# wenyuqing/panacea

Measured on NVIDIA H100. Metric: UNet denoise-steps/s (6-view x 8-frame latent, CFG-doubled eps-eval + guidance + Euler update), higher is better.
Workload: dtype bf16

## Files before the change

### panacea_b200/csrc/attn_fa.cu

```cuda
#include "common.cuh"
#include "ptx.cuh"
#include "operand.cuh"
#include "../../include/panacea_b200.h"

namespace pn {

constexpr int FA_THREADS = 288;
constexpr int FA_TILE_BYTES = 128 * 128;
constexpr int FA_XTILE_BYTES = 128 * 32;
constexpr int FA_MAX_KEYS = 128;
constexpr int FA_QBOX = 8;

template <int D>
struct FaL {
  static constexpr int STAGES = 3;
  static constexpr int XB = D == 64 ? 0 : FA_XTILE_BYTES;
  static constexpr int Q = 0;
  static constexpr int QX = FA_TILE_BYTES;
  static constexpr int KV = FA_TILE_BYTES + XB;
  static constexpr int STAGE_BYTES = 2 * FA_TILE_BYTES + 2 * XB;
  static constexpr int BAR = KV + STAGES * STAGE_BYTES;
  static constexpr int TOTAL = BAR + 128 + 1024;
};

struct FaParams {
  CUtensorMap mapQ;
  CUtensorMap mapK;
  CUtensorMap mapV;
  CUtensorMap mapQx, mapKx, mapVx;
  int heads;
  int F, H, V, W;
  int q_rowmajor;
  int qw, qh, tiles_x, tiles_y;
  int tiles_per_group;
  int kw, kh, kv_rows, kv_yblocks;
  int kv_views[8][2];
  int kv_view_count[8];
  int kv_frame_div;
  float scale_log2;
  __nv_bfloat16* out;
  long long out_ld;
};

template <int D, int N>
__global__ void __launch_bounds__(FA_THREADS, 1) attn_fa_kernel(const __grid_constant__ FaParams p) {
  static_assert(N % 16 == 0 && N >= 16 && N <= FA_MAX_KEYS, "a key block is a whole number of K = 16 steps of P V");
  using L = FaL<D>;
  constexpr int STAGES = L::STAGES;
  constexpr int GROUPS = N / 8;
  constexpr int KSTEPS = N / 16;
  extern __shared__ uint8_t smem_raw[];
  uint8_t* smem = smem_align1024(smem_raw);
  uint64_t* bars = reinterpret_cast<uint64_t*>(smem + L::BAR);
  uint64_t* q_full = bars;
  uint64_t* kv_full = bars + 1;
  uint64_t* kv_empty = bars + 1 + STAGES;

  const int warp = threadIdx.x >> 5;
  const int lane = threadIdx.x & 31;

  {
    uint4* z = reinterpret_cast<uint4*>(smem);
    for (int i = threadIdx.x; i < L::BAR / 16; i += FA_THREADS) z[i] = make_uint4(0, 0, 0, 0);
    fence_proxy_async_smem();
  }
  if (threadIdx.x == 0) {
    mbar_init(q_full, 1);
    for (int i = 0; i < STAGES; ++i) { mbar_init(&kv_full[i], 1); mbar_init(&kv_empty[i], 2); }
    fence_barrier_init();
  }
  __syncthreads();

  int item = blockIdx.x;
  const int ti = item % p.tiles_per_group; item /= p.tiles_per_group;
  const int head = item % p.heads; item /= p.heads;
  const int view = item % p.V;
  const int frame = item / p.V;
  const int nblk = p.kv_view_count[view] * p.kv_yblocks;

  if (warp == 8) {
    const uint32_t row_bytes = D == 80 ? 160u : 128u;
    const uint32_t kv_bytes = (uint32_t)p.kv_rows * row_bytes;
    if (elect_one()) {
      tma_prefetch_desc(&p.mapQ);
      tma_prefetch_desc(&p.mapK);
      tma_prefetch_desc(&p.mapV);
      if (p.q_rowmajor) {
        const int t0 = ti * 128;
        const int rows = min(128, p.H * p.W - t0);
        mbar_arrive_expect_tx(q_full, (uint32_t)rows * row_bytes);
        for (int r = 0; r < rows; r += FA_QBOX) {
          const int y = (t0 + r) / p.W, x = t0 + r - y * p.W;
          tma_load_5d(smem + L::Q + r * 128, &p.mapQ, q_full, head * D, x, view, y, frame);
          if (D == 80) tma_load_5d(smem + L::QX + r * 32, &p.mapQx, q_full, head * D + 64, x, view, y, frame);
        }
      } else {
        mbar_arrive_expect_tx(q_full, (uint32_t)(p.qw * p.qh) * row_bytes);
        const int x0 = (ti % p.tiles_x) * p.qw, y0 = (ti / p.tiles_x) * p.qh;
        tma_load_5d(smem + L::Q, &p.mapQ, q_full, head * D, x0, view, y0, frame);
        if (D == 80) tma_load_5d(smem + L::QX, &p.mapQx, q_full, head * D + 64, x0, view, y0, frame);
      }
    }
    const int kv_frame = frame / p.kv_frame_div;
    int vi = 0, yb = 0;
    for (int j = 0; j < nblk; ++j) {
      const int st = j % STAGES;
      const int kvv = p.kv_views[view][vi];
      mbar_wait(&kv_empty[st], (uint32_t)(((j / STAGES) & 1) ^ 1));
      if (elect_one()) {
        uint8_t* sK = smem + L::KV + st * L::STAGE_BYTES;
        mbar_arrive_expect_tx(&kv_full[st], 2 * kv_bytes);
        tma_load_5d(sK, &p.mapK, &kv_full[st], head * D, 0, kvv, yb * p.kh, kv_frame);
        tma_load_5d(sK + FA_TILE_BYTES, &p.mapV, &kv_full[st], head * D, 0, kvv, yb * p.kh, kv_frame);
        if (D == 80) {
          tma_load_5d(sK + 2 * FA_TILE_BYTES, &p.mapKx, &kv_full[st], head * D + 64, 0, kvv, yb * p.kh, kv_frame);
          tma_load_5d(sK + 2 * FA_TILE_BYTES + L::XB, &p.mapVx, &kv_full[st], head * D + 64, 0, kvv, yb * p.kh, kv_frame);
        }
      }
      if (++yb == p.kv_yblocks) { yb = 0; ++vi; }
    }
    return;
  }

  const int wg = warp >> 2;
  const int quad = lane & 3;
  const uint32_t base = smem_u32(smem);
  const uint64_t dQ = wgmma_desc(base + L::Q + wg * 64 * 128, 16, 1024, kSw128);
  const uint64_t dQx = wgmma_desc(base + L::QX + wg * 64 * 32, 16, 256, kSw32);
  const uint64_t dK0 = wgmma_desc(base + L::KV, 16, 1024, kSw128);
  const uint64_t dV0 = wgmma_desc(base + L::KV + FA_TILE_BYTES, 1024, 1024, kSw128);
  const uint64_t dKx0 = wgmma_desc(base + L::KV + 2 * FA_TILE_BYTES, 16, 256, kSw32);
  const uint64_t dVx0 = wgmma_desc(base + L::KV + 2 * FA_TILE_BYTES + L::XB, 256, 256, kSw32);
  constexpr uint64_t STAGE_STEP = L::STAGE_BYTES >> 4;
  const float c = p.scale_log2;
  const bool mask = p.kv_rows < N;

  float o[32], ox[8];
#pragma unroll
  for (int i = 0; i < 32; ++i) o[i] = 0.f;
#pragma unroll
  for (int i = 0; i < 8; ++i) ox[i] = 0.f;
  float m_run[2] = {-INFINITY, -INFINITY}, l_run[2] = {0.f, 0.f};
  float s[N / 2];
  uint32_t pa[KSTEPS][4];
  float alpha[2];

  auto issue_s = [&](int st) {
#pragma unroll
    for (int k = 0; k < 4; ++k) wgmma_ss<N>(s, dQ + 2 * k, dK0 + STAGE_STEP * st + 2 * k, k > 0 ? 1u : 0u);
    if (D == 80) wgmma_ss<N>(s, dQx, dKx0 + STAGE_STEP * st, 1u);
    wgmma_commit();
  };
  auto issue_pv = [&](int st) {
#pragma unroll
    for (int kk = 0; kk < KSTEPS; ++kk) {
      wgmma_rs_tb<64>(o, pa[kk], dV0 + STAGE_STEP * st + kk * (2048 >> 4), 1u);
      if (D == 80) wgmma_rs_tb<16>(ox, pa[kk], dVx0 + STAGE_STEP * st + kk * (512 >> 4), 1u);
    }
    wgmma_commit();
  };
  auto softmax = [&]() {
    float mx[2] = {-INFINITY, -INFINITY};
#pragma unroll
    for (int jj = 0; jj < GROUPS; ++jj) {
#pragma unroll
      for (int e = 0; e < 4; ++e) {
        if (jj >= GROUPS - 2 && mask && 8 * jj + 2 * quad + (e & 1) >= p.kv_rows) s[4 * jj + e] = -INFINITY;
        mx[e >> 1] = fmaxf(mx[e >> 1], s[4 * jj + e]);
      }
    }
    float mc[2];
#pragma unroll
    for (int h = 0; h < 2; ++h) {
      mx[h] = fmaxf(mx[h], __shfl_xor_sync(0xffffffffu, mx[h], 1));
      mx[h] = fmaxf(mx[h], __shfl_xor_sync(0xffffffffu, mx[h], 2));
      const float m_new = fmaxf(m_run[h], mx[h]);
      alpha[h] = ex2_approx((m_run[h] - m_new) * c);
      m_run[h] = m_new;
      mc[h] = m_new * c;
    }
    float rs[2] = {0.f, 0.f};
#pragma unroll
    for (int jj = 0; jj < GROUPS; ++jj) {
#pragma unroll
      for (int e = 0; e < 4; ++e) {
        const float x = fmaf(s[4 * jj + e], c, -mc[e >> 1]);
        const float v = ex2_approx(x);
        s[4 * jj + e] = v;
        rs[e >> 1] += v;
      }
    }
#pragma unroll
    for (int h = 0; h < 2; ++h) l_run[h] = l_run[h] * alpha[h] + rs[h];
  };
  auto rescale_and_pack = [&]() {
#pragma unroll
    for (int i = 0; i < 32; ++i) o[i] *= alpha[(i >> 1) & 1];
    if (D == 80) {
#pragma unroll
      for (int i = 0; i < 8; ++i) ox[i] *= alpha[(i >> 1) & 1];
    }
#pragma unroll
    for (int jj = 0; jj < GROUPS; ++jj) {
#pragma unroll
      for (int h = 0; h < 2; ++h) pa[jj >> 1][(jj & 1) * 2 + h] = pack_bf16x2(s[4 * jj + 2 * h], s[4 * jj + 2 * h + 1]);
    }
  };
  auto pv_retired = [&](int st) {
    wgmma_fence_regs(o);
    if (D == 80) wgmma_fence_regs(ox);
#pragma unroll
    for (int kk = 0; kk < KSTEPS; ++kk) wgmma_fence_regs(pa[kk]);
    if ((threadIdx.x & 127) == 0) mbar_arrive(&kv_empty[st]);
  };

  mbar_wait(q_full, 0);
  mbar_wait(&kv_full[0], 0);
  wgmma_fence();
  issue_s(0);
  wgmma_wait<0>();
  wgmma_fence_regs(s);
  softmax();
  rescale_and_pack();
  for (int j = 1; j < nblk; ++j) {
    const int st = j % STAGES, prev = (j - 1) % STAGES;
    mbar_wait(&kv_full[st], (uint32_t)((j / STAGES) & 1));
    wgmma_fence();
    issue_s(st);
    issue_pv(prev);
    wgmma_wait<0>();
    wgmma_fence_regs(s);
    pv_retired(prev);
    softmax();
    rescale_and_pack();
  }
  wgmma_fence();
  issue_pv((nblk - 1) % STAGES);
  wgmma_wait<0>();
  pv_retired((nblk - 1) % STAGES);

#pragma unroll
  for (int h = 0; h < 2; ++h) {
    float l = l_run[h];
    l += __shfl_xor_sync(0xffffffffu, l, 1);
    l += __shfl_xor_sync(0xffffffffu, l, 2);
    const float inv = 1.f / l;
    const int row = wg * 64 + (warp & 3) * 16 + (lane >> 2) + 8 * h;
    int x, y;
    if (p.q_rowmajor) {
      const int t = ti * 128 + row;
      y = t / p.W;
      x = t - y * p.W;
    } else {
      if (row >= p.qw * p.qh) continue;
      const int yy = row / p.qw, xx = row - yy * p.qw;
      x = (ti % p.tiles_x) * p.qw + xx;
      y = (ti / p.tiles_x) * p.qh + yy;
    }
    if (x >= p.W || y >= p.H) continue;
    const long long token = (((long long)frame * p.H + y) * p.V + view) * p.W + x;
    __nv_bfloat16* dst = p.out + token * p.out_ld + head * D + 2 * quad;
#pragma unroll
    for (int jj = 0; jj < 8; ++jj)
      *reinterpret_cast<uint32_t*>(dst + 8 * jj) = pack_bf16x2(o[4 * jj + 2 * h] * inv, o[4 * jj + 2 * h + 1] * inv);
    if (D == 80) {
#pragma unroll
      for (int jj = 0; jj < 2; ++jj)
        *reinterpret_cast<uint32_t*>(dst + 64 + 8 * jj) = pack_bf16x2(ox[4 * jj + 2 * h] * inv, ox[4 * jj + 2 * h + 1] * inv);
    }
  }
}

template <int D>
void (*const fa_kernels[FA_MAX_KEYS / 16])(FaParams) = {attn_fa_kernel<D, 16>, attn_fa_kernel<D, 32>, attn_fa_kernel<D, 48>,
                                                        attn_fa_kernel<D, 64>, attn_fa_kernel<D, 80>, attn_fa_kernel<D, 96>,
                                                        attn_fa_kernel<D, 112>, attn_fa_kernel<D, 128>};

}

using namespace pn;

extern "C" int pn_attention(const pn_attn_args* a, int operand_mode, void* stream_v) {
  PN_OPERAND_MODES(Modes, operand_mode, "pn_attention", PN_OPERAND_BF16, PN_OPERAND_SPLIT3, PN_OPERAND_F32);
  if (operand_mode != PN_OPERAND_BF16) return attention_f32(a, operand_mode, stream_v);
  if (a == nullptr) return fail(PN_ERR_INVALID, "pn_attention: null args");
  PN_REQUIRE(a->q && a->k && a->v && a->out, "pn_attention: null tensor pointer");
  PN_REQUIRE(a->head_dim == 64 || a->head_dim == 80, "pn_attention: head_dim %d unsupported (64 or 80)", a->head_dim);
  const int FA_D = a->head_dim;
  PN_REQUIRE(a->heads > 0 && a->F > 0 && a->H > 0 && a->V > 0 && a->V <= 8 && a->W > 0, "pn_attention: bad query geometry");
  PN_REQUIRE(a->Hk > 0 && a->Vk > 0 && a->Vk <= 8 && a->Wk > 0 && a->kv_frame_div > 0, "pn_attention: bad key geometry");
  PN_REQUIRE(a->q_ld % 8 == 0 && a->kv_ld % 8 == 0 && a->out_ld % 8 == 0, "pn_attention: token strides must be multiples of 8");
  PN_REQUIRE(a->q_ld >= a->heads * FA_D && a->kv_ld >= a->heads * FA_D && a->out_ld >= a->heads * FA_D,
             "pn_attention: token stride smaller than heads*64");

  FaParams p;
  std::memset(&p, 0, sizeof(p));
  p.heads = a->heads;
  p.F = (int)a->F; p.H = (int)a->H; p.V = (int)a->V; p.W = (int)a->W;
  p.qw = (int)(a->W <= 128 ? a->W : 128);
  p.qh = 128 / p.qw;
  if (p.qh > a->H) p.qh = (int)a->H;
  if (p.qh < 1) p.qh = 1;
  p.tiles_x = (int)((a->W + p.qw - 1) / p.qw);
  p.tiles_y = (int)((a->H + p.qh - 1) / p.qh);
  p.q_rowmajor = a->W % FA_QBOX == 0 && a->W < 128 && p.qw * p.qh < 128 && a->H > p.qh;
  PN_REQUIRE(a->Wk <= FA_MAX_KEYS, "pn_attention: key view width %lld > %d unsupported", (long long)a->Wk, FA_MAX_KEYS);
  p.kw = (int)a->Wk;
  int kh = FA_MAX_KEYS / p.kw;
  if (kh > a->Hk) kh = (int)a->Hk;
  while (kh > 1 && (a->Hk % kh) != 0) --kh;
  p.kh = kh;
  p.kv_rows = p.kw * p.kh;
  p.kv_yblocks = (int)(a->Hk / p.kh);
  for (int v = 0; v < a->V; ++v) {
    const int cnt = a->kv_view_count[v];
    PN_REQUIRE(cnt >= 1 && cnt <= 2, "pn_attention: kv_view_count[%d]=%d must be 1 or 2", v, cnt);
    p.kv_view_count[v] = cnt;
    for (int i = 0; i < cnt; ++i) {
      PN_REQUIRE(a->kv_views[v][i] >= 0 && a->kv_views[v][i] < a->Vk, "pn_attention: kv view out of range");
      p.kv_views[v][i] = a->kv_views[v][i];
    }
  }
  p.kv_frame_div = a->kv_frame_div;
  p.scale_log2 = a->scale * 1.4426950408889634f;
  p.out = reinterpret_cast<__nv_bfloat16*>(a->out);
  p.out_ld = a->out_ld;

  const uint64_t chq = (uint64_t)a->heads * FA_D;
  {
    const uint64_t dims[5] = {chq, (uint64_t)a->W, (uint64_t)a->V, (uint64_t)a->H, (uint64_t)a->F};
    const uint64_t ld = (uint64_t)a->q_ld;
    const uint64_t str[4] = {ld, ld * a->W, ld * a->W * a->V, ld * a->W * a->V * a->H};
    const uint32_t bw = p.q_rowmajor ? FA_QBOX : p.qw, bh = p.q_rowmajor ? 1 : p.qh;
    const uint32_t box[5] = {64u, bw, 1u, bh, 1u};
    int rc = cached_tmap_bf16(&p.mapQ, a->q, 5, dims, str, box, 128);
    if (rc != PN_OK) return rc;
    if (FA_D == 80) {
      const uint32_t boxx[5] = {16u, bw, 1u, bh, 1u};
      rc = cached_tmap_bf16(&p.mapQx, a->q, 5, dims, str, boxx, 32);
      if (rc != PN_OK) return rc;
    }
  }
  {
    const uint64_t Fk = (uint64_t)((a->F + a->kv_frame_div - 1) / a->kv_frame_div);
    const uint64_t dims[5] = {chq, (uint64_t)a->Wk, (uint64_t)a->Vk, (uint64_t)a->Hk, Fk};
    const uint64_t ld = (uint64_t)a->kv_ld;
    const uint64_t str[4] = {ld, ld * a->Wk, ld * a->Wk * a->Vk, ld * a->Wk * a->Vk * a->Hk};
    const uint32_t box[5] = {64u, (uint32_t)p.kw, 1u, (uint32_t)p.kh, 1u};
    int rc = cached_tmap_bf16(&p.mapK, a->k, 5, dims, str, box, 128);
    if (rc != PN_OK) return rc;
    rc = cached_tmap_bf16(&p.mapV, a->v, 5, dims, str, box, 128);
    if (rc != PN_OK) return rc;
    if (FA_D == 80) {
      const uint32_t boxx[5] = {16u, (uint32_t)p.kw, 1u, (uint32_t)p.kh, 1u};
      rc = cached_tmap_bf16(&p.mapKx, a->k, 5, dims, str, boxx, 32);
      if (rc != PN_OK) return rc;
      rc = cached_tmap_bf16(&p.mapVx, a->v, 5, dims, str, boxx, 32);
      if (rc != PN_OK) return rc;
    }
  }
  p.tiles_per_group = p.q_rowmajor ? (int)((a->H * a->W + 127) / 128) : p.tiles_x * p.tiles_y;
  const long long items = (long long)p.tiles_per_group * a->heads * a->V * a->F;
  PN_REQUIRE(items > 0 && items < (1ll << 31), "pn_attention: too many query tiles");
  const int n_idx = (p.kv_rows + 15) / 16 - 1;
  void (*kern)(FaParams) = FA_D == 80 ? fa_kernels<80>[n_idx] : fa_kernels<64>[n_idx];
  const size_t smem_total = FA_D == 80 ? FaL<80>::TOTAL : FaL<64>::TOTAL;
  {
    const int rc = ensure_dyn_smem(reinterpret_cast<const void*>(kern), smem_total);
    if (rc != PN_OK) return rc;
  }
  kern<<<(unsigned)items, FA_THREADS, smem_total, reinterpret_cast<cudaStream_t>(stream_v)>>>(p);
  PN_CHECK_CUDA(cudaGetLastError());
  return PN_OK;
}
```

Measured before the change: 4.208.

## Make attention CTAs persistent over query tiles when KV fits one block

When every query's key/value set fits in a single block, each CTA now processes several query tiles of the same head/view/frame. K/V is loaded once and Q tiles stream through extra slots carved from the unused KV stages, with their own full/empty barriers. The S=QK^T of the next tile overlaps the PV and store of the current one. This is meant to remove repeated K/V loads and per-CTA launch and prologue cost. The risks are lower parallelism, since the grid shrinks to about two CTAs per SM, and extra barrier complexity.

```diff
diff --git a/panacea_b200/csrc/attn_fa.cu b/panacea_b200/csrc/attn_fa.cu
--- a/panacea_b200/csrc/attn_fa.cu
+++ b/panacea_b200/csrc/attn_fa.cu
@@ -10,6 +10,7 @@
 constexpr int FA_XTILE_BYTES = 128 * 32;
 constexpr int FA_MAX_KEYS = 128;
 constexpr int FA_QBOX = 8;
+constexpr int FA_STREAM_CTAS = 2 * 132;
 
 template <int D>
 struct FaL {
@@ -21,6 +22,13 @@
   static constexpr int STAGE_BYTES = 2 * FA_TILE_BYTES + 2 * XB;
   static constexpr int BAR = KV + STAGES * STAGE_BYTES;
   static constexpr int TOTAL = BAR + 128 + 1024;
+  static constexpr int QSLOTS = 1 + 2 * (STAGES - 1);
+  __device__ static int q_off(int i) {
+    return i == 0 ? Q : KV + ((i + 1) >> 1) * STAGE_BYTES + ((i + 1) & 1) * FA_TILE_BYTES;
+  }
+  __device__ static int qx_off(int i) {
+    return i == 0 ? QX : KV + ((i + 1) >> 1) * STAGE_BYTES + 2 * FA_TILE_BYTES + ((i + 1) & 1) * XB;
+  }
 };
 
 struct FaParams {
@@ -33,6 +41,7 @@
   int q_rowmajor;
   int qw, qh, tiles_x, tiles_y;
   int tiles_per_group;
+  int tiles_per_cta;
   int kw, kh, kv_rows, kv_yblocks;
   int kv_views[8][2];
   int kv_view_count[8];
@@ -53,8 +62,10 @@
   uint8_t* smem = smem_align1024(smem_raw);
   uint64_t* bars = reinterpret_cast<uint64_t*>(smem + L::BAR);
   uint64_t* q_full = bars;
-  uint64_t* kv_full = bars + 1;
-  uint64_t* kv_empty = bars + 1 + STAGES;
+  uint64_t* q_empty = bars + L::QSLOTS;
+  uint64_t* kv_full = bars + 2 * L::QSLOTS;
+  uint64_t* kv_empty = bars + 2 * L::QSLOTS + STAGES;
+  static_assert((2 * L::QSLOTS + 2 * STAGES) * 8 <= 128, "barriers fit their 128 bytes");
 
   const int warp = threadIdx.x >> 5;
   const int lane = threadIdx.x & 31;
@@ -65,18 +76,22 @@
     fence_proxy_async_smem();
   }
   if (threadIdx.x == 0) {
-    mbar_init(q_full, 1);
+    for (int i = 0; i < L::QSLOTS; ++i) { mbar_init(&q_full[i], 1); mbar_init(&q_empty[i], 2); }
     for (int i = 0; i < STAGES; ++i) { mbar_init(&kv_full[i], 1); mbar_init(&kv_empty[i], 2); }
     fence_barrier_init();
   }
   __syncthreads();
 
+  const int ctas_per_group = (p.tiles_per_group + p.tiles_per_cta - 1) / p.tiles_per_cta;
   int item = blockIdx.x;
-  const int ti = item % p.tiles_per_group; item /= p.tiles_per_group;
+  const int ti0 = (item % ctas_per_group) * p.tiles_per_cta; item /= ctas_per_group;
   const int head = item % p.heads; item /= p.heads;
   const int view = item % p.V;
   const int frame = item / p.V;
+  const int ntiles = min(p.tiles_per_cta, p.tiles_per_group - ti0);
   const int nblk = p.kv_view_count[view] * p.kv_yblocks;
+  const bool kv_once = nblk == 1;
+  const int qslots = kv_once ? L::QSLOTS : 1;
 
   if (warp == 8) {
     const uint32_t row_bytes = D == 80 ? 160u : 128u;
@@ -85,39 +100,49 @@
       tma_prefetch_desc(&p.mapQ);
       tma_prefetch_desc(&p.mapK);
       tma_prefetch_desc(&p.mapV);
-      if (p.q_rowmajor) {
-        const int t0 = ti * 128;
-        const int rows = min(128, p.H * p.W - t0);
-        mbar_arrive_expect_tx(q_full, (uint32_t)rows * row_bytes);
-        for (int r = 0; r < rows; r += FA_QBOX) {
-          const int y = (t0 + r) / p.W, x = t0 + r - y * p.W;
-          tma_load_5d(smem + L::Q + r * 128, &p.mapQ, q_full, head * D, x, view, y, frame);
-          if (D == 80) tma_load_5d(smem + L::QX + r * 32, &p.mapQx, q_full, head * D + 64, x, view, y, frame);
+    }
+    const int kv_frame = frame / p.kv_frame_div;
+    int g = 0;
+    for (int t = 0; t < ntiles; ++t) {
+      const int slot = t % qslots, ti = ti0 + t;
+      mbar_wait(&q_empty[slot], (uint32_t)(((t / qslots) & 1) ^ 1));
+      if (elect_one()) {
+        uint8_t* sQ = smem + L::q_off(slot);
+        uint8_t* sQx = smem + L::qx_off(slot);
+        if (p.q_rowmajor) {
+          const int t0 = ti * 128;
+          const int rows = min(128, p.H * p.W - t0);
+          mbar_arrive_expect_tx(&q_full[slot], (uint32_t)rows * row_bytes);
+          for (int r = 0; r < rows; r += FA_QBOX) {
+            const int y = (t0 + r) / p.W, x = t0 + r - y * p.W;
+            tma_load_5d(sQ + r * 128, &p.mapQ, &q_full[slot], head * D, x, view, y, frame);
+            if (D == 80) tma_load_5d(sQx + r * 32, &p.mapQx, &q_full[slot], head * D + 64, x, view, y, frame);
+          }
+        } else {
+          mbar_arrive_expect_tx(&q_full[slot], (uint32_t)(p.qw * p.qh) * row_bytes);
+          const int x0 = (ti % p.tiles_x) * p.qw, y0 = (ti / p.tiles_x) * p.qh;
+          tma_load_5d(sQ, &p.mapQ, &q_full[slot], head * D, x0, view, y0, frame);
+          if (D == 80) tma_load_5d(sQx, &p.mapQx, &q_full[slot], head * D + 64, x0, view, y0, frame);
         }
-      } else {
-        mbar_arrive_expect_tx(q_full, (uint32_t)(p.qw * p.qh) * row_bytes);
-        const int x0 = (ti % p.tiles_x) * p.qw, y0 = (ti / p.tiles_x) * p.qh;
-        tma_load_5d(smem + L::Q, &p.mapQ, q_full, head * D, x0, view, y0, frame);
-        if (D == 80) tma_load_5d(smem + L::QX, &p.mapQx, q_full, head * D + 64, x0, view, y0, frame);
-      }
-    }
-    const int kv_frame = frame / p.kv_frame_div;
-    int vi = 0, yb = 0;
-    for (int j = 0; j < nblk; ++j) {
-      const int st = j % STAGES;
-      const int kvv = p.kv_views[view][vi];
-      mbar_wait(&kv_empty[st], (uint32_t)(((j / STAGES) & 1) ^ 1));
-      if (elect_one()) {
-        uint8_t* sK = smem + L::KV + st * L::STAGE_BYTES;
-        mbar_arrive_expect_tx(&kv_full[st], 2 * kv_bytes);
-        tma_load_5d(sK, &p.mapK, &kv_full[st], head * D, 0, kvv, yb * p.kh, kv_frame);
-        tma_load_5d(sK + FA_TILE_BYTES, &p.mapV, &kv_full[st], head * D, 0, kvv, yb * p.kh, kv_frame);
-        if (D == 80) {
-          tma_load_5d(sK + 2 * FA_TILE_BYTES, &p.mapKx, &kv_full[st], head * D + 64, 0, kvv, yb * p.kh, kv_frame);
-          tma_load_5d(sK + 2 * FA_TILE_BYTES + L::XB, &p.mapVx, &kv_full[st], head * D + 64, 0, kvv, yb * p.kh, kv_frame);
+      }
+      if (kv_once && t > 0) continue;
+      int vi = 0, yb = 0;
+      for (int j = 0; j < nblk; ++j, ++g) {
+        const int st = g % STAGES;
+        const int kvv = p.kv_views[view][vi];
+        mbar_wait(&kv_empty[st], (uint32_t)(((g / STAGES) & 1) ^ 1));
+        if (elect_one()) {
+          uint8_t* sK = smem + L::KV + st * L::STAGE_BYTES;
+          mbar_arrive_expect_tx(&kv_full[st], 2 * kv_bytes);
+          tma_load_5d(sK, &p.mapK, &kv_full[st], head * D, 0, kvv, yb * p.kh, kv_frame);
+          tma_load_5d(sK + FA_TILE_BYTES, &p.mapV, &kv_full[st], head * D, 0, kvv, yb * p.kh, kv_frame);
+          if (D == 80) {
+            tma_load_5d(sK + 2 * FA_TILE_BYTES, &p.mapKx, &kv_full[st], head * D + 64, 0, kvv, yb * p.kh, kv_frame);
+            tma_load_5d(sK + 2 * FA_TILE_BYTES + L::XB, &p.mapVx, &kv_full[st], head * D + 64, 0, kvv, yb * p.kh, kv_frame);
+          }
         }
-      }
-      if (++yb == p.kv_yblocks) { yb = 0; ++vi; }
+        if (++yb == p.kv_yblocks) { yb = 0; ++vi; }
+      }
     }
     return;
   }
@@ -125,8 +150,6 @@
   const int wg = warp >> 2;
   const int quad = lane & 3;
   const uint32_t base = smem_u32(smem);
-  const uint64_t dQ = wgmma_desc(base + L::Q + wg * 64 * 128, 16, 1024, kSw128);
-  const uint64_t dQx = wgmma_desc(base + L::QX + wg * 64 * 32, 16, 256, kSw32);
   const uint64_t dK0 = wgmma_desc(base + L::KV, 16, 1024, kSw128);
   const uint64_t dV0 = wgmma_desc(base + L::KV + FA_TILE_BYTES, 1024, 1024, kSw128);
   const uint64_t dKx0 = wgmma_desc(base + L::KV + 2 * FA_TILE_BYTES, 16, 256, kSw32);
@@ -136,16 +159,22 @@
   const bool mask = p.kv_rows < N;
 
   float o[32], ox[8];
-#pragma unroll
-  for (int i = 0; i < 32; ++i) o[i] = 0.f;
-#pragma unroll
-  for (int i = 0; i < 8; ++i) ox[i] = 0.f;
-  float m_run[2] = {-INFINITY, -INFINITY}, l_run[2] = {0.f, 0.f};
+  float m_run[2], l_run[2];
   float s[N / 2];
   uint32_t pa[KSTEPS][4];
   float alpha[2];
-
-  auto issue_s = [&](int st) {
+  auto reset = [&]() {
+#pragma unroll
+    for (int i = 0; i < 32; ++i) o[i] = 0.f;
+#pragma unroll
+    for (int i = 0; i < 8; ++i) ox[i] = 0.f;
+    m_run[0] = m_run[1] = -INFINITY;
+    l_run[0] = l_run[1] = 0.f;
+    wgmma_fence_regs(o);
+    if (D == 80) wgmma_fence_regs(ox);
+  };
+
+  auto issue_s = [&](uint64_t dQ, uint64_t dQx, int st) {
 #pragma unroll
     for (int k = 0; k < 4; ++k) wgmma_ss<N>(s, dQ + 2 * k, dK0 + STAGE_STEP * st + 2 * k, k > 0 ? 1u : 0u);
     if (D == 80) wgmma_ss<N>(s, dQx, dKx0 + STAGE_STEP * st, 1u);
@@ -193,13 +222,15 @@
 #pragma unroll
     for (int h = 0; h < 2; ++h) l_run[h] = l_run[h] * alpha[h] + rs[h];
   };
-  auto rescale_and_pack = [&]() {
+  auto rescale = [&]() {
 #pragma unroll
     for (int i = 0; i < 32; ++i) o[i] *= alpha[(i >> 1) & 1];
     if (D == 80) {
 #pragma unroll
       for (int i = 0; i < 8; ++i) ox[i] *= alpha[(i >> 1) & 1];
     }
+  };
+  auto pack = [&]() {
 #pragma unroll
     for (int jj = 0; jj < GROUPS; ++jj) {
 #pragma unroll
@@ -211,64 +242,99 @@
     if (D == 80) wgmma_fence_regs(ox);
 #pragma unroll
     for (int kk = 0; kk < KSTEPS; ++kk) wgmma_fence_regs(pa[kk]);
-    if ((threadIdx.x & 127) == 0) mbar_arrive(&kv_empty[st]);
-  };
-
-  mbar_wait(q_full, 0);
+    if (!kv_once && (threadIdx.x & 127) == 0) mbar_arrive(&kv_empty[st]);
+  };
+  auto store_tile = [&](int ti) {
+#pragma unroll
+    for (int h = 0; h < 2; ++h) {
+      float l = l_run[h];
+      l += __shfl_xor_sync(0xffffffffu, l, 1);
+      l += __shfl_xor_sync(0xffffffffu, l, 2);
+      const float inv = 1.f / l;
+      const int row = wg * 64 + (warp & 3) * 16 + (lane >> 2) + 8 * h;
+      int x, y;
+      if (p.q_rowmajor) {
+        const int t = ti * 128 + row;
+        y = t / p.W;
+        x = t - y * p.W;
+      } else {
+        if (row >= p.qw * p.qh) continue;
+        const int yy = row / p.qw, xx = row - yy * p.qw;
+        x = (ti % p.tiles_x) * p.qw + xx;
+        y = (ti / p.tiles_x) * p.qh + yy;
+      }
+      if (x >= p.W || y >= p.H) continue;
+      const long long token = (((long long)frame * p.H + y) * p.V + view) * p.W + x;
+      __nv_bfloat16* dst = p.out + token * p.out_ld + head * D + 2 * quad;
+#pragma unroll
+      for (int jj = 0; jj < 8; ++jj)
+        *reinterpret_cast<uint32_t*>(dst + 8 * jj) = pack_bf16x2(o[4 * jj + 2 * h] * inv, o[4 * jj + 2 * h + 1] * inv);
+      if (D == 80) {
+#pragma unroll
+        for (int jj = 0; jj < 2; ++jj)
+          *reinterpret_cast<uint32_t*>(dst + 64 + 8 * jj) = pack_bf16x2(ox[4 * jj + 2 * h] * inv, ox[4 * jj + 2 * h + 1] * inv);
+      }
+    }
+  };
+  auto q_desc = [&](int slot) { return wgmma_desc(base + L::q_off(slot) + wg * 64 * 128, 16, 1024, kSw128); };
+  auto qx_desc = [&](int slot) { return wgmma_desc(base + L::qx_off(slot) + wg * 64 * 32, 16, 256, kSw32); };
+  auto q_release = [&](int slot) {
+    if ((threadIdx.x & 127) == 0) mbar_arrive(&q_empty[slot]);
+  };
+
+  reset();
+  mbar_wait(&q_full[0], 0);
   mbar_wait(&kv_full[0], 0);
   wgmma_fence();
-  issue_s(0);
+  issue_s(q_desc(0), qx_desc(0), 0);
   wgmma_wait<0>();
   wgmma_fence_regs(s);
   softmax();
-  rescale_and_pack();
-  for (int j = 1; j < nblk; ++j) {
-    const int st = j % STAGES, prev = (j - 1) % STAGES;
-    mbar_wait(&kv_full[st], (uint32_t)((j / STAGES) & 1));
-    wgmma_fence();
-    issue_s(st);
-    issue_pv(prev);
-    wgmma_wait<0>();
-    wgmma_fence_regs(s);
-    pv_retired(prev);
-    softmax();
-    rescale_and_pack();
+  rescale();
+  pack();
+  if (kv_once) q_release(0);
+  int st_last = 0;
+  if (kv_once) {
+    for (int t = 0; t + 1 < ntiles; ++t) {
+      const int next = (t + 1) % qslots;
+      const uint64_t dQ = q_desc(next), dQx = qx_desc(next);
+      mbar_wait(&q_full[next], (uint32_t)(((t + 1) / qslots) & 1));
+      wgmma_fence();
+      issue_s(dQ, dQx, 0);
+      issue_pv(0);
+      wgmma_wait<0>();
+      wgmma_fence_regs(s);
+      pv_retired(0);
+      q_release(next);
+      store_tile(ti0 + t);
+      reset();
+      softmax();
+      rescale();
+      pack();
+    }
+  } else {
+    const uint64_t dQ = q_desc(0), dQx = qx_desc(0);
+    for (int j = 1; j < nblk; ++j) {
+      const int st = j % STAGES, prev = (j - 1) % STAGES;
+      mbar_wait(&kv_full[st], (uint32_t)((j / STAGES) & 1));
+      wgmma_fence();
+      issue_s(dQ, dQx, st);
+      issue_pv(prev);
+      wgmma_wait<0>();
+      wgmma_fence_regs(s);
+      pv_retired(prev);
+      softmax();
+      rescale();
+      pack();
+    }
+    st_last = (nblk - 1) % STAGES;
   }
   wgmma_fence();
-  issue_pv((nblk - 1) % STAGES);
+  issue_pv(st_last);
   wgmma_wait<0>();
-  pv_retired((nblk - 1) % STAGES);
-
-#pragma unroll
-  for (int h = 0; h < 2; ++h) {
-    float l = l_run[h];
-    l += __shfl_xor_sync(0xffffffffu, l, 1);
-    l += __shfl_xor_sync(0xffffffffu, l, 2);
-    const float inv = 1.f / l;
-    const int row = wg * 64 + (warp & 3) * 16 + (lane >> 2) + 8 * h;
-    int x, y;
-    if (p.q_rowmajor) {
-      const int t = ti * 128 + row;
-      y = t / p.W;
-      x = t - y * p.W;
-    } else {
-      if (row >= p.qw * p.qh) continue;
-      const int yy = row / p.qw, xx = row - yy * p.qw;
-      x = (ti % p.tiles_x) * p.qw + xx;
-      y = (ti / p.tiles_x) * p.qh + yy;
-    }
-    if (x >= p.W || y >= p.H) continue;
-    const long long token = (((long long)frame * p.H + y) * p.V + view) * p.W + x;
-    __nv_bfloat16* dst = p.out + token * p.out_ld + head * D + 2 * quad;
-#pragma unroll
-    for (int jj = 0; jj < 8; ++jj)
-      *reinterpret_cast<uint32_t*>(dst + 8 * jj) = pack_bf16x2(o[4 * jj + 2 * h] * inv, o[4 * jj + 2 * h + 1] * inv);
-    if (D == 80) {
-#pragma unroll
-      for (int jj = 0; jj < 2; ++jj)
-        *reinterpret_cast<uint32_t*>(dst + 64 + 8 * jj) = pack_bf16x2(ox[4 * jj + 2 * h] * inv, ox[4 * jj + 2 * h + 1] * inv);
-    }
-  }
+  pv_retired(st_last);
+  if (!kv_once) q_release(0);
+  store_tile(ti0 + ntiles - 1);
 }
 
 template <int D>
@@ -360,7 +426,11 @@
     }
   }
   p.tiles_per_group = p.q_rowmajor ? (int)((a->H * a->W + 127) / 128) : p.tiles_x * p.tiles_y;
-  const long long items = (long long)p.tiles_per_group * a->heads * a->V * a->F;
+  bool one_block = p.kv_yblocks == 1;
+  for (int v = 0; v < a->V; ++v) one_block = one_block && p.kv_view_count[v] == 1;
+  const long long tiles = (long long)p.tiles_per_group * a->heads * a->V * a->F;
+  p.tiles_per_cta = one_block ? (int)((tiles + FA_STREAM_CTAS - 1) / FA_STREAM_CTAS) : 1;
+  const long long items = (long long)((p.tiles_per_group + p.tiles_per_cta - 1) / p.tiles_per_cta) * a->heads * a->V * a->F;
   PN_REQUIRE(items > 0 && items < (1ll << 31), "pn_attention: too many query tiles");
   const int n_idx = (p.kv_rows + 15) / 16 - 1;
   void (*kern)(FaParams) = FA_D == 80 ? fa_kernels<80>[n_idx] : fa_kernels<64>[n_idx];
```

After: 4.273 (median of 6 runs). +1.5%, better.
